# MaaniGhaffari/cvo-rgbd

Measured on AMD Instinct MI355X. Metric: frame-pair registrations/sec, higher is better.
Workload: dtype f32; 1 GPU; BASELINE configs[1] shape: 64 distinct synthetic 10000x10000 RGB-D cloud pairs (xyz + 5-dim colour) per align_many call, cvo align() to convergence, clouds resident in HBM; points_fixed=10000, points_moving=10000, mode=cvo, batch=64

## Files before the change

### cvo-rgbd_amd/csrc/cvo_capi.cpp

```cpp
#include "cvo_internal.h"

using namespace cvo_dev;
using namespace cvo_impl;

namespace cvo_impl {

int fail(cvo_hip_ctx *ctx, int code, const char *msg)
{
    if (ctx) ctx->err = msg;
    return code;
}

static std::atomic<bool> g_engine_debug{false};
bool engine_debug_on() { return g_engine_debug.load(std::memory_order_relaxed); }

namespace {
struct OptDef {
    const char *key;
    const char *env;
    int env_kind;
    double env_value;
};
const OptDef kOptions[] = {
    {"graph_capture", "CVO_HIP_GRAPH", 1, 1.0},           {"no_graph", "CVO_HIP_NO_GRAPH", 1, 1.0},
// ... 822 lines not shown
    else if (is("kept_pack")) *value = !o.no_pack;
    else if (is("matches_combine")) *value = o.matches_combine;
    else if (is("scan_chunk")) *value = o.scan_chunk;
    else if (is("list_margin")) *value = o.list_margin;
    else if (is("record_narrow")) *value = o.record_narrow;
    else if (is("list_stale_max")) *value = o.list_stale_max;
    else if (is("final_mirror")) *value = !o.no_final_mirror;
    else if (is("twist_on_shared_gpu")) *value = o.twist_on_shared_gpu;
    else if (is("comm_debug")) *value = o.comm_debug;
    else if (is("wait_policy")) *value = o.wait_policy;
    else if (is("acvo_runs")) *value = !o.no_acvo_run;
    else if (is("tail_alone")) *value = o.tail_alone;
    else if (is("tail_handovers")) *value = (double)ctx->tail_handovers;
    else if (is("run_restart")) *value = !o.no_restart;
    else if (is("side_builds")) *value = !o.no_side_builds;
    else if (is("run_build_at")) *value = o.run_build_at;
    else if (is("side_builds_launched")) *value = (double)ctx->side_builds_launched;
    else if (is("alone_max")) *value = o.alone_max;
    else if (is("run_timeouts")) *value = (double)ctx->run_timeouts;
    else if (is("list_grows")) *value = (double)ctx->list_grows;
    else if (is("async_builds_named")) *value = (double)ctx->async_stats[0];
    else if (is("async_stalls")) *value = (double)ctx->async_stats[1];
    else if (is("run_aborts")) *value = (double)ctx->run_aborts;
    else if (is("no_run_backoff")) *value = ctx->no_run_backoff;
    else return CVO_HIP_ERR_INVALID;
    return CVO_HIP_OK;
}

long long cvo_hip_get_mirror_retries(void) { return mirror_retries().load(std::memory_order_relaxed); }

int cvo_hip_synchronize(cvo_hip_ctx *ctx)
{
    cvo_lock::Api api_guard;
    if (!ctx) return CVO_HIP_ERR_INVALID;
    HIP_TRY(ctx, hipStreamSynchronize(ctx->stream));
    return CVO_HIP_OK;
}


}
```

### cvo-rgbd_amd/csrc/cvo_device.h

```cpp
#pragma once

#include <hip/hip_runtime.h>
#include <hip/hip_ext.h>
#include <stddef.h>
#include <stdint.h>

#include "cvo_hip.h"
#include "se3_math.hpp"

namespace cvo_dev {

constexpr int FEAT_STRIDE = 8;
constexpr int FEAT_INDEX_SLOT = 5;

constexpr int BLOCK = 256;
constexpr int TILES_PER_WAVE = 4;
constexpr int ROWS_PER_WAVE = 16 * TILES_PER_WAVE;
constexpr int ROWS_PER_TILE = 4 * ROWS_PER_WAVE;
constexpr float PAD_BIG = 1.0e30f;
constexpr int PROC_BLOCKS = 1024;
constexpr int PROC_WAVES = PROC_BLOCKS * 4;

constexpr int NSUB = 256;
constexpr int PROC_PARTS = PROC_BLOCKS / NSUB;
// ... 600 lines not shown
        s->run_hint = (nnz > 0.0f && nnz < 1.0e9f) ? (int32_t)fminf(1.105f * nnz * (q * q) * (w * w), 2.0e9f) : 0;
        s->r_last = r_now;
    }
    if (p.async_self) {
        const float s_xx = reuse_slack(s->t, s->center, s->xmax, s->y0max, 0.0f), s_yy = reuse_slack(s->t, s->center, s->xmax, s->y0max, 1.0f);
        plan_self_async_one<0>(s, p, r_now * 1.0001f + s_xx, p.list_margin, 0.0f, b.sf_fresh[0], b.sf_failed[0], b.sf_inflight[0]);
        plan_self_async_one<1>(s, p, r_now * 1.0001f + s_yy, p.list_margin, s_yy - s_xx, b.sf_fresh[1], b.sf_failed[1], b.sf_inflight[1]);
    }
}

CVO_HD void count_async_plan(DevHead *dst, const DevHead *planned, const DevParams &p)
{
    if (p.async_xy && planned->xy_target >= 0) dst->async_stat[0] += 1;
    if ((p.async_xy || p.async_self) && planned->stall) dst->async_stat[1] += 1;
}

size_t filter_smem_bytes(int jt);
struct PrepareInit {
    int32_t on;
    float R[9], T[3], ell, ell_max;
    int32_t iter, n_fixed, done;
    float center[3], xmax, y0max;
};
struct KeptView {
    const uint2 *kept_ij;
    const float *kept_a;
    const uint32_t *kept_cnt;
    const DevState *st;
    uint32_t kept_wcap;
    int nblk;
    int kept_packed;
    unsigned kept_ebase;
};
#define CVO_GLOBAL __attribute__((address_space(1)))
typedef unsigned u32x2_t __attribute__((ext_vector_type(2)));
typedef float f32x4_t __attribute__((ext_vector_type(4)));
CVO_HD float4 apply_tf(const float *Rt, const float *t, const float4 p)
{
    float4 o;
    o.x = ((Rt[0] * p.x + Rt[1] * p.y) + Rt[2] * p.z) + t[0];
    o.y = ((Rt[3] * p.x + Rt[4] * p.y) + Rt[5] * p.z) + t[1];
    o.z = ((Rt[6] * p.x + Rt[7] * p.y) + Rt[8] * p.z) + t[2];
    o.w = p.w;
    return o;
}

// ... 210 lines not shown
void launch_pose_matches(const MatchArgs &a, bool combine, hipStream_t s);

constexpr int SCAN_TF = 16;
constexpr int SCAN_CHUNK = 4096;
constexpr int SCAN_MAX_POINTS = 65536;
struct ScanArgs {
    const float4 *pos_a;
    const float *feat_a;
    const float4 *seg_a;
    const float4 *pos_b;
    const float *feat_b;
    const float4 *seg_b;
    const float *tf;
    double *partials;
    double *out;
    KernConsts kc;
    int nseg_a, nseg_b;
    int nblk;
    int count;
};
void launch_pose_scan(const ScanArgs &a, int weight, hipStream_t s);

void launch_prepare(DevState *st, const DevParams &prm, hipStream_t s, uint32_t *build_masks = nullptr, const PrepareInit *init = nullptr);
void launch_filter(const FilterArgs &a, dim3 grid, hipStream_t s, hipEvent_t ev_start = nullptr,
                   hipEvent_t ev_stop = nullptr);
void launch_process(int mode, const ProcessArgs &a, hipStream_t s, hipEvent_t ev_start = nullptr,
                    hipEvent_t ev_stop = nullptr);
void launch_post_flow(const PostFlowArgs &a, hipStream_t s);
void launch_post_step(const PostStepArgs &a, hipStream_t s);
void launch_filter_group(const FilterArgs *a, int n, hipStream_t s);
void launch_process_group(int mode, const ProcessArgs *a, int n, hipStream_t s, hipEvent_t ev_start = nullptr,
                          hipEvent_t ev_stop = nullptr);
void launch_post_flow_group(const PostFlowArgs *a, int n, hipStream_t s);
void launch_post_step_group(const PostStepArgs *a, int n, hipStream_t s);
void launch_step_twist_group(const ProcessArgs *a, int n, hipStream_t s, hipEvent_t ev_start = nullptr,
                             hipEvent_t ev_stop = nullptr);
constexpr int STEP_TWIST_ROWS_DIV = 4;

enum TKernel { TK_FILTER = 0, TK_FILTER_GROUP, TK_FLOW, TK_FLOW_MATLAB, TK_STEP, TK_SELF, TK_SELF2, TK_STEP_TWIST,
               TK_FLOW_BUILD, TK_FLOW_BUILD3, TK_FLOW_BUILD6, TK_POST_FLOW, TK_POST_STEP,
               TK_HFLOW_BUILD, TK_HFLOW_BUILD6, TK_HSTEP_TWIST, TK_RUN , TK_RUN_ACVO ,
               TK_SIDE_FILTER, TK_SIDE_RECORD ,
               TK_FLOW_D2  };
constexpr int QP_PARITY = 1 << 8, QP_HEAD = 1 << 9, QP_MASK = 0xff;
struct TLaunch {
    int kernel;
// ... 13 lines not shown
```

### cvo-rgbd_amd/csrc/cvo_engine.cpp

```cpp
#include "cvo_internal.h"

using namespace cvo_dev;
using namespace cvo_impl;

namespace cvo_impl {

bool fusable(const cvo_hip_ctx *c) { return !c->profiling && !multi_rank(c) && !(c->prm.color_scale > 0.0f); }



struct EngineProfile {
    std::mutex mu;
    bool on = false;
    double flow_ms = 0.0, flow_slots = 0.0;
    long long flow_launches = 0;
    std::vector<float> dur_us, period_us;
    std::vector<int> slots;
};
EngineProfile *engine_profile()
{
    static EngineProfile *p = new EngineProfile;
    return p;
}

// ... 10 lines not shown
            (acvo ? !c->allow_async_self : !c->allow_run))
            return false;
        pairs = std::max(pairs, (double)c->fixed.n * (double)c->moving.n);
    }
    const size_t few = acvo ? (pairs <= 1.6e7 ? 12 : (pairs <= 5.0e7 ? 4 : (pairs <= 1.2e8 ? 4 : 0)))
                            : (pairs <= 1.6e7 ? 12 : (pairs <= 5.0e7 ? 8 : (pairs <= 2.0e8 ? 4 : 0)));
    if (const int force = pending.front()->ctx->opt.alone_max) return pending.size() <= (size_t)force;
    return pending.size() <= few;
}

struct Engine {
    int device = 0;
    hipStream_t s = nullptr;
    TableBuf tab;
    PlanCache plans;
    bool in_use = false;

    AlignJob *member[ENGINE_SLOTS] = {};
    std::vector<RecOp> ops[ENGINE_SLOTS];
    Slot slot[ENGINE_SLOTS];
    struct Retire { hipEvent_t ev = nullptr; std::vector<AlignJob *> jobs; };
    std::vector<Retire> retiring;
    hipEvent_t ev[4] = {};
    long long launched = 0, checked = 0;
    int zdim = 0;
    bool crowded = true, use_graph = true, dirty = true, failed = false;
    int batch_len = kEngineBatch;
    bool narrow = false;
    bool narrow_merge = false;
    int narrow_blocks = 0;
    bool wind_down = false;
    std::vector<TLaunch> plan;
    struct FlowEv { hipEvent_t a, b; int live; };
    std::vector<FlowEv> flow_ev;
    long long n_batches[5] = {}, n_replans = 0, n_inserts = 0, n_sends = 0;
    double t_replan = 0, t_insert = 0, t_launch = 0, t_finish = 0, t_wait = 0, t_collect = 0, t_idle_at = 0;
    static double now_ms() { return std::chrono::duration<double, std::milli>(std::chrono::steady_clock::now().time_since_epoch()).count(); }

    int create(int dev)
    {
        device = dev;
        if (hipSetDevice(dev) != hipSuccess) return -1;
        if (hipStreamCreateWithFlags(&s, hipStreamNonBlocking) != hipSuccess) return -1;
        if (tab.init(ENGINE_SLOTS, s) != 0) return -1;
        for (auto &e : ev)
            if (hipEventCreateWithFlags(&e, hipEventDisableTiming) != hipSuccess) return -1;
        return 0;
    }

    int live() const { int n = 0; for (AlignJob *j : member) n += j != nullptr; return n; }
    bool idle() const { return live() == 0 && retiring.empty() && launched == checked; }

    static int nblk_for(int z)
    {
        constexpr int budget = 2048;
        int nblk = 64;
        while (nblk < PROC_BLOCKS && nblk * 2 <= (budget + z / 2) / std::max(1, z)) nblk *= 2;
        return nblk;
// ... 3 lines not shown
    {
        j->rc = rc;
        j->phase = 2;
        j->in_group = false;
        j->ctx->loop_stream = nullptr;
        j->ctx->crowded = false;
        j->ctx->lone = true;
        j->ctx->proc_blocks = j->ctx->proc_blocks_default;
    }

    void fail_all(const char *msg, std::deque<AlignJob *> &pending)
    {
        failed = true;
        (void)hipStreamSynchronize(s);
        for (AlignJob *&j : member)
            if (j) { finish_job(j, fail(j->ctx, CVO_HIP_ERR_HIP, msg)); j = nullptr; }
        for (auto &r : retiring) {
            for (AlignJob *j : r.jobs) finish_job(j, fail(j->ctx, CVO_HIP_ERR_HIP, msg));
            if (r.ev) (void)hipEventDestroy(r.ev);
        }
        retiring.clear();
        for (AlignJob *j : pending) { j->rc = fail(j->ctx, CVO_HIP_ERR_HIP, msg); j->phase = 2; }
        pending.clear();
        for (int z = 0; z < ENGINE_SLOTS; ++z) slot[z].active = 0;
        (void)tab.sync(slot, s, 0);
        (void)hipStreamSynchronize(s);
        launched = checked = 0;
    }

    int insert(AlignJob *j, int z)
    {
        cvo_hip_ctx *c = j->ctx;
        c->loop_stream = s;
        c->crowded = crowded;
        c->lone = false;
        j->in_group = true;
        int rc = CVO_HIP_OK;
        if (j->phase == 3) {
            int32_t zero = 0;
            std::memcpy(&c->st_host[kPollSlots].done, &zero, sizeof(zero));
            if (hipMemcpyAsync(reinterpret_cast<char *>(c->st) + offsetof(DevState, done), &c->st_host[kPollSlots].done,
                               sizeof(zero), hipMemcpyHostToDevice, s) != hipSuccess)
                rc = fail(c, CVO_HIP_ERR_HIP, "resume failed");
            *c->done_mirror = 0;
            launch_prepare(c->st, loop_params(c), s, tab.masks());
            j->phase = 0;
        } else {
            rc = job_begin(*j);
        }
        if (rc) { finish_job(j, rc); return rc; }
        if (j->phase != 0) {
            Retire r;
            if (hipEventCreateWithFlags(&r.ev, hipEventDisableTiming) != hipSuccess || hipEventRecord(r.ev, s) != hipSuccess) {
                finish_job(j, fail(c, CVO_HIP_ERR_HIP, "event failed"));
                return CVO_HIP_ERR_HIP;
            }
            r.jobs.push_back(j);
            retiring.push_back(r);
            return CVO_HIP_OK;
        }
        member[z] = j;
        ops[z].clear();
        dirty = true;
        (void)tab.arm(s);
        return CVO_HIP_OK;
    }

    int replan()
    {
        int n = 0;
        for (int z = 0; z < ENGINE_SLOTS; ++z) n += member[z] != nullptr;
        int zd = 1;
        while (zd < n) zd *= 2;
        if (n > 16 && n <= 24) zd = 24;
        for (int z = ENGINE_SLOTS - 1, hole = 0; z >= zd; --z) {
            if (!member[z]) continue;
            while (member[hole]) ++hole;
            member[hole] = member[z]; member[z] = nullptr;
            ops[hole].swap(ops[z]); ops[z].clear();
        }
        const bool regeom = zd != zdim;
        zdim = zd;
        const int nblk = (narrow && narrow_blocks > 0) ? std::min(narrow_blocks, nblk_for(zdim)) : nblk_for(zdim);
        int merge_max = 2;
        std::vector<const std::vector<RecOp> *> po;
        std::vector<Slot *> ps;
        for (int z = 0; z < ENGINE_SLOTS; ++z)
// ... 9 lines not shown
                c->allow_merge = allow;
                if (rc) return rc;
            }
            std::memset(&slot[z], 0, sizeof(Slot));
            slot[z].active = 1;
            po.push_back(&ops[z]);
            ps.push_back(&slot[z]);
        }
        if (!plan_fused(po, ps, zdim, plan)) return CVO_HIP_ERR_INVALID;
        for (int z = 0; z < ENGINE_SLOTS; ++z)
            if (member[z]) set_build_masks(slot[z], plan, tab.masks(), z);
        const int nq = po.empty() ? 0 : (int)po[0]->size();
        if (tab.sync(slot, s, nq) != 0) return CVO_HIP_ERR_HIP;
        ++n_replans;
        dirty = false;
        return CVO_HIP_OK;
    }

    void collect_stopped()
    {
        Retire r;
        for (int z = 0; z < ENGINE_SLOTS; ++z) {
            AlignJob *j = member[z];
            if (!j || *(volatile int32_t *)j->ctx->done_mirror == RUNNING) continue;
            if (hipMemcpyAsync(&j->ctx->st_host[0], j->ctx->st, sizeof(DevState), hipMemcpyDeviceToHost, s) != hipSuccess) {
                finish_job(j, fail(j->ctx, CVO_HIP_ERR_HIP, "state copy failed"));
            } else {
                r.jobs.push_back(j);
            }
            member[z] = nullptr;
            ops[z].clear();
            dirty = true;
        }
        if (r.jobs.empty()) return;
        if (hipEventCreateWithFlags(&r.ev, hipEventDisableTiming) != hipSuccess || hipEventRecord(r.ev, s) != hipSuccess) {
            for (AlignJob *j : r.jobs) finish_job(j, fail(j->ctx, CVO_HIP_ERR_HIP, "event failed"));
            if (r.ev) (void)hipEventDestroy(r.ev);
            return;
        }
        retiring.push_back(r);
    }

    bool finish_arrived(std::deque<AlignJob *> &pending, bool block)
    {
        bool moved = false;
        while (!retiring.empty()) {
            Retire &r = retiring.front();
            const hipError_t q = block ? hipEventSynchronize(r.ev) : hipEventQuery(r.ev);
            if (q == hipErrorNotReady) break;
            block = false;
// ... 46 lines not shown
                        }
                    }
                    launch_table(tab.dev, l, s);
                }
            return hipGetLastError() == hipSuccess ? CVO_HIP_OK : CVO_HIP_ERR_HIP;
        }
        return run_plan(tab.dev, plans, plan, s, use_graph, batch);
    }

    bool pump(std::deque<AlignJob *> &pending, int want)
    {
        if (failed) return false;
        if (hipSetDevice(device) != hipSuccess) { fail_all("hipSetDevice failed", pending); return true; }
        bool moved = false;
        while (checked < launched) {
            const hipError_t q = hipEventQuery(ev[checked % 4]);
            if (q == hipErrorNotReady) break;
            if (q != hipSuccess) { fail_all("fused poll failed", pending); return true; }
            ++checked;
            { const double t0 = now_ms(); collect_stopped(); t_collect += now_ms() - t0; }
            moved = true;
        }
        { const double t0 = now_ms(); if (finish_arrived(pending, false)) moved = true; t_finish += now_ms() - t0; }
        while (!pending.empty() && live() < std::min(want, (int)ENGINE_SLOTS)) {
            AlignJob *j = pending.front();
            pending.pop_front();
            int z = 0;
            while (member[z]) ++z;
            { const double t0 = now_ms(); insert(j, z); t_insert += now_ms() - t0; }
            moved = true;
        }
        constexpr long long depth = 2;
        while (live() > 0 && launched - checked < depth && !wind_down) {
            if (dirty) {
                const double t0 = now_ms();
                const int rc = replan();
                t_replan += now_ms() - t0;
                if (rc) { fail_all("fused launch recording failed", pending); return true; }
            }
            const double t_l0 = now_ms();
            const int rc_launch = launch_one_batch();
            if (rc_launch != CVO_HIP_OK ||
                hipEventRecord(ev[launched % 4], s) != hipSuccess) {
                fail_all("fused launch failed", pending);
                return true;
            }
            t_launch += now_ms() - t_l0;
            ++launched;
            ++n_batches[zdim >= 16 ? 4 : (zdim >= 8 ? 3 : (zdim >= 4 ? 2 : (zdim >= 2 ? 1 : 0)))];
            moved = true;
        }
        if (live() == 0 && dirty && launched == checked) {
            if (replan() != CVO_HIP_OK) { fail_all("table update failed", pending); return true; }
// ... 58 lines not shown
    if (!e->flow_ev.empty()) {
        EngineProfile *pr = engine_profile();
        std::lock_guard<std::mutex> plock(pr->mu);
        for (size_t q = 0; q < e->flow_ev.size(); ++q) {
            auto &fe = e->flow_ev[q];
            float ms = 0.f, gap = 0.f;
            if (hipEventSynchronize(fe.b) == hipSuccess && hipEventElapsedTime(&ms, fe.a, fe.b) == hipSuccess) {
                pr->flow_ms += ms; pr->flow_launches++; pr->flow_slots += fe.live;
                if (q + 1 < e->flow_ev.size() && hipEventElapsedTime(&gap, fe.a, e->flow_ev[q + 1].a) != hipSuccess) gap = 0.f;
                if (pr->dur_us.size() < (size_t)1 << 20) {
                    pr->dur_us.push_back(ms * 1e3f); pr->period_us.push_back(gap * 1e3f); pr->slots.push_back(fe.live);
                }
            }
        }
        for (auto &fe : e->flow_ev) {
            (void)hipEventDestroy(fe.a);
            (void)hipEventDestroy(fe.b);
        }
        e->flow_ev.clear();
    }
    std::lock_guard<std::mutex> lock(*engine_mutex());
    if (engine_debug_on())
        fprintf(stderr, "[cvo_hip] engine %p: batches at zdim 1/2/4/8/16: %lld %lld %lld %lld %lld, replans %lld, "
                "graph captures %lld hits %lld; host ms: insert %.2f replan %.2f launch %.2f collect %.2f finish %.2f wait %.2f\n",
                (void *)e, e->n_batches[0], e->n_batches[1], e->n_batches[2],
                e->n_batches[3], e->n_batches[4], e->n_replans, e->plans.captures, e->plans.hits,
                e->t_insert, e->t_replan, e->t_launch, e->t_collect, e->t_finish, e->t_wait);
    e->t_insert = e->t_replan = e->t_launch = e->t_collect = e->t_finish = e->t_wait = 0;
    for (long long &v : e->n_batches) v = 0;
    e->n_replans = 0;
    e->launched = e->checked = 0;
    e->in_use = false;
}


}

extern "C" {

int cvo_hip_align_many(cvo_hip_ctx **ctxs, cvo_hip_state **states, int *n_iters, int count)
{
    cvo_lock::Api api_guard;
    if (count < 0 || (count > 0 && (!ctxs || !states))) return CVO_HIP_ERR_INVALID;
    const bool dbg_many = engine_debug_on();
    const double t_many0 = Engine::now_ms();
    struct Tell { double t0; int n; ~Tell() { if (engine_debug_on()) fprintf(stderr, "[cvo_hip] align_many(%d): %.2f ms\n", n, Engine::now_ms() - t0); } } tell{t_many0, count};
    std::vector<AlignJob> jobs((size_t)count);
    for (int i = 0; i < count; ++i) {
        if (!ctxs[i] || !states[i]) return CVO_HIP_ERR_INVALID;
        for (int k = 0; k < i; ++k)
            if (ctxs[k] == ctxs[i]) return CVO_HIP_ERR_INVALID;
        jobs[i].ctx = ctxs[i];
        jobs[i].s = states[i];
// ... 73 lines not shown
                            for (int z = 0; z < ENGINE_SLOTS; ++z) e->ops[z].clear();
                        }
                    if (dbg_many && (left != dbg_left || (int)narrow != dbg_narrow)) { dbg_left = left; dbg_narrow = (int)narrow; fprintf(stderr, "[cvo_hip]   %.2f ms: %d left (narrow %d settled %d)\n", Engine::now_ms() - t_many0, left, (int)narrow, (int)settled); }
                    (void)settled;
                    if (tail_ok && left > 0 && left <= tail_k && narrow) {
                        for (Engine *e : engines) e->wind_down = true;
                        if (dbg_many) {
                            fprintf(stderr, "[cvo_hip]   tail: %d registrations left after %.2f ms, slots done:", left, Engine::now_ms() - t_many0);
                            for (Engine *e : engines)
                                for (AlignJob *j : e->member)
                                    if (j) fprintf(stderr, " %d", *(volatile int32_t *)j->ctx->progress_mirror);
                            fprintf(stderr, "\n");
                        }
                    }
                }
                for (Engine *e : engines) {
                    if (e->wind_down) {
                        const size_t before = leavers.size();
                        e->release_members(leavers);
                        if (leavers.size() != before) {
                            moved = true;
                            if (dbg_many) fprintf(stderr, "[cvo_hip]   tail: %zu registrations leave engine %p after %.2f ms\n", leavers.size() - before, (void *)e, Engine::now_ms() - t_many0);
                        }
                    }
                    if (e->pump(pending, share)) moved = true;
                    if (!e->idle()) any = true;
                    else if (dbg_many && e->t_idle_at == 0) {
                        e->t_idle_at = Engine::now_ms();
                        fprintf(stderr, "[cvo_hip]   engine %p idle after %.2f ms\n", (void *)e, e->t_idle_at - t_many0);
                    }
                }
                if (!any && pending.empty()) break;
                bool alive = false;
                for (Engine *e : engines) alive = alive || !e->failed;
                if (!alive) break;
                if (!moved)
                    for (Engine *e : engines)
                        if (!e->idle() && !e->failed) { e->wait_oldest(pending); break; }
            }
            for (Engine *e : engines) { e->wind_down = false; e->narrow = false; e->batch_len = kEngineBatch; engine_release(e); }
        }
        for (int i = 0; i < count; ++i)
            if (jobs[i].phase == 2 && jobs[i].rc && !first_err) first_err = jobs[i].rc;
    }
    std::vector<char> cont((size_t)count, 0);
    for (AlignJob *j : leavers) {
// ... 92 lines not shown
```

### cvo-rgbd_amd/csrc/cvo_internal.h

```cpp
#pragma once
#include "cvo_hip.h"

#include <hip/hip_runtime.h>

#include <algorithm>
#include <atomic>
#include <chrono>
#include <cmath>
#include <cstddef>
#include <cstdint>
#include <cstdio>
#include <cstdlib>
#include <cstring>
#include <deque>
#include <memory>
#include <mutex>
#include <new>
#include <string>
#include <thread>
#include <vector>

#include "cvo_cloud.h"
#include "cvo_comm.h"
#include "cvo_device.h"
// ... 191 lines not shown
    int tail_alone = 8;
    int alone_max = 0;
    int engines_force = 0;
    int narrow_blocks = 0;
    bool narrow_merge = false;
    int engine_crowd = 2;
    int engine_merge_max = 2;
    double list_init = 0.0;
    float list_margin = -1.0f;
    bool record_narrow = true;
    float list_stale_max = 3.0f;
    int run_cand = 0;
    double mailbox_timeout_s = 5.0;
    double run_timeout_ms = 0.0;
    int run_fault = 0;
    int wait_policy = 0;
};

struct cvo_hip_ctx {
    CtxOptions opt;
    int no_run_backoff = 0;
    long long side_builds_launched = 0;
    long long tail_handovers = 0;
    long long run_aborts = 0;
    int list_stats[3] = {0, 0, 0};
    int async_stats[2] = {0, 0};
    long long list_grows = 0;
    long long run_timeouts = 0;
    int device = 0;
    hipStream_t stream = nullptr;
    bool own_stream = false;
    cvo_hip_params prm{};
    DevParams dprm{};
    Cloud fixed, moving;
    Cloud scratch_a, scratch_b;
    DevState *st = nullptr;
    DevHead *st2 = nullptr;
    bool head_mode = false;
    bool allow_head = true;
    DevState *st_host = nullptr;
    int32_t *done_mirror = nullptr;
    int32_t *progress_mirror = nullptr;
    DevHead *final_mirror = nullptr;
    int32_t *run_mirror = nullptr;
    int32_t *hint_mirror = nullptr;
    int32_t *side_mirror = nullptr;
// ... 146 lines not shown
int enqueue_iterations(cvo_hip_ctx *ctx, int count, int tag0, int trace_cap);
void drop_graphs(cvo_hip_ctx *ctx);
TLaunch mk_launch(int kernel, int q, unsigned gx, unsigned gz, unsigned smem = 0);
bool plan_lone(const std::vector<RecOp> &ops, Slot &slot, std::vector<TLaunch> &plan, const bool allow_head, bool *head_mode,
               std::vector<TLaunch> *pre = nullptr, std::vector<TLaunch> *side = nullptr);
void set_build_masks(Slot &slot, const std::vector<TLaunch> &plan, uint32_t *masks, int z);
bool plan_fused(const std::vector<const std::vector<RecOp> *> &ops, const std::vector<Slot *> &slots, int zdim, std::vector<TLaunch> &plan);
int run_plan(const Slot *tab, PlanCache &cache, const std::vector<TLaunch> &plan, hipStream_t s, bool use_graph, int iterations,
             const std::vector<TLaunch> *pre = nullptr);
int record_iteration(cvo_hip_ctx *ctx, std::vector<RecOp> &ops, int trace_cap);
int prepare_lone_plan(cvo_hip_ctx *ctx, int trace_cap);
int launch_batch(cvo_hip_ctx *ctx, int tag0, int trace_cap, bool with_run = false, int slots = kBatch, bool small_run = false, bool two_runs = false);
constexpr int kNoRunBackoff = 64;
constexpr int kBigRunBackoff = 16;
constexpr int kShortBatch = 2;
constexpr int kRunBatchSlots = 2;
int zero_counters(cvo_hip_ctx *ctx);
int push_state_fields(cvo_hip_ctx *ctx, size_t off, size_t bytes);
int push_pose_fields(cvo_hip_ctx *ctx, const DevHead *img, bool with_consts);
int enqueue_flow_reduce(cvo_hip_ctx *ctx, const CommTable *comm);
int fetch_red(cvo_hip_ctx *ctx, int off, int count, double *out);
void decide_scheme(cvo_hip_ctx *ctx);
std::atomic<long long> &mirror_retries();
int job_begin(AlignJob &j);
int job_finish(AlignJob &j);
int job_continue_alone(AlignJob &j);
int job_pump(AlignJob &j, bool block);

}
```

### cvo-rgbd_amd/csrc/cvo_job.cpp

```cpp
#include "cvo_internal.h"

using namespace cvo_dev;
using namespace cvo_impl;

namespace cvo_impl {

void decide_scheme(cvo_hip_ctx *ctx)
{
    const bool small_pair = (double)ctx->fixed.n * (double)ctx->moving.n <= 2.5e7;
    if (!ctx->proc_blocks_forced)
        ctx->proc_blocks = ctx->proc_blocks_default = small_pair ? PROC_BLOCKS / 2 : PROC_BLOCKS;
    ctx->use_async = ctx->allow_async && !ctx->crowded && !ctx->profiling && !multi_rank(ctx) &&
                     !(ctx->prm.color_scale > 0.0f) &&
                     (double)ctx->fixed.n * (double)ctx->moving.n <= 2.0e8;
    ctx->use_async_self = ctx->use_async && ctx->allow_async_self && ctx->lone &&
                          ctx->prm.mode == CVO_HIP_MODE_ACVO;
    const double npairs = (double)ctx->fixed.n * (double)ctx->moving.n;
    if (ctx->use_async_self && !ctx->proc_blocks_forced)
        ctx->proc_blocks = ctx->proc_blocks_default = npairs <= 6.0e7 ? PROC_BLOCKS / 8 : PROC_BLOCKS / 4;
    if (!ctx->proc_blocks_forced && !ctx->use_async_self && ctx->use_async && ctx->lone && ctx->allow_head &&
        ctx->prm.mode == CVO_HIP_MODE_CVO)
    {
        const bool runs = runs_allowed(ctx) && ctx->fixed.np <= 65536 && ctx->moving.np <= 65536;
        ctx->proc_blocks = ctx->proc_blocks_default =
            npairs <= 2.5e7 ? PROC_BLOCKS / 4 : (npairs <= (runs ? 6.0e7 : 1.5e8) ? PROC_BLOCKS / 2 : PROC_BLOCKS);
    }
}

std::atomic<long long> &mirror_retries()
{
    static std::atomic<long long> n{0};
    return n;
}

int job_begin(AlignJob &j)
{
    cvo_hip_ctx *ctx = j.ctx;
    cvo_hip_state *s = j.s;
    HIP_TRY(ctx, hipSetDevice(ctx->device));
    {
        const int rcm = mailboxes_usable(ctx);
        if (rcm) return rcm;
    }
    const cvo_hip_params &p = ctx->prm;
    if (ctx->no_run_backoff > 0) --ctx->no_run_backoff;
    if (p.mode == CVO_HIP_MODE_ACVO) {
        s->ell = p.ell_init;
        s->ell_max = p.ell_max_init;
    }
    *ctx->done_mirror = 0;
    *ctx->progress_mirror = 0;
    *ctx->run_mirror = 0;
    *ctx->hint_mirror = -1;
    *ctx->side_mirror = 0;
    j.side_seen = 0;
    j.side_launched = 0;
    if (ctx->final_mirror) ctx->final_mirror->done = RUNNING;
    if (!j.trace) j.trace_cap = 0;
// ... 4 lines not shown
        HIP_TRY(ctx, hipMalloc((void **)&ctx->trace_dev, (size_t)j.trace_cap * sizeof(cvo_hip_trace)));
        ctx->trace_dev_cap = j.trace_cap;
    }
    if (j.trace_cap > 0)
        HIP_TRY(ctx, hipMemsetAsync(ctx->trace_dev, 0, (size_t)j.trace_cap * sizeof(cvo_hip_trace),
                                    loop_stream(ctx)));
    PrepareInit in{};
    {
        DevState *h = &ctx->st_host[kPollSlots];
        const int rcg = fill_filter_geometry(ctx, h);
        if (rcg) return rcg;
        in.on = 1;
        std::memcpy(in.R, s->R, sizeof(in.R));
        std::memcpy(in.T, s->T, sizeof(in.T));
        in.ell = s->ell;
        in.ell_max = s->ell_max;
        in.iter = s->iter;
        in.n_fixed = h->n_fixed;
        for (int q = 0; q < 3; ++q) in.center[q] = h->center[q];
        in.xmax = h->xmax; in.y0max = h->y0max;
        in.done = p.max_iter <= 0 ? DONE_MAX_ITER : RUNNING;
    }
    decide_scheme(ctx);
    launch_prepare(ctx->st, loop_params(ctx), loop_stream(ctx), (!j.in_group && ctx->table.raw) ? ctx->table.masks() : nullptr, &in);
    HIP_TRY(ctx, hipGetLastError());
    ctx->have_tf = true;
    const int prc = prepare_buffers(ctx);
    if (prc) return prc;
    ctx->head_mode = false;
    if (!j.in_group && !ctx->profiling && !host_reduce(ctx)) {
        const int rc2 = prepare_lone_plan(ctx, j.trace_cap);
        if (rc2) return rc2;
    }
    j.enq = j.batches = j.checked = 0;
    j.runs_enq = 0;
    j.run_waiting = false;
    j.spec_pending = false;
    j.executed_base = 0;
    const int g_call = std::max(8, std::min(ctx->run_g_max, ctx->run_g_call));
    ctx->run_nnz_max = g_call * RUN_BLOCK * (RUN_R + RUN_L);
    ctx->run_small_max = 3 * RUN_G_SMALL * RUN_BLOCK;
    if (ctx->prm.mode == CVO_HIP_MODE_ACVO) {
        ctx->run_nnz_max = (int)(0.8 * g_call * RUN_BLOCK * RUN_A);
        ctx->run_small_max = (int)(0.8 * 2 * RUN_G_SMALL * RUN_BLOCK);
    }
    if (ctx->big_run_backoff > 0) --ctx->big_run_backoff;
    if (ctx->opt.run_cand > 0) ctx->run_nnz_max = ctx->opt.run_cand;
    j.phase = p.max_iter <= 0 ? 1 : 0;
    if (j.phase == 1) {
        HIP_TRY(ctx, hipMemcpyAsync(&ctx->st_host[0], ctx->st, sizeof(DevState), hipMemcpyDeviceToHost,
                                    loop_stream(ctx)));
        HIP_TRY(ctx, hipEventRecord(ctx->poll_ev[0], loop_stream(ctx)));
    }
    return CVO_HIP_OK;
}

int job_continue_alone(AlignJob &j)
{
    cvo_hip_ctx *ctx = j.ctx;
    HIP_TRY(ctx, hipSetDevice(ctx->device));
    j.in_group = false;
    ctx->loop_stream = nullptr;
    ctx->crowded = false;
    ctx->lone = true;
    ctx->proc_blocks = ctx->proc_blocks_default;
    if (ctx->no_run_backoff > 0) --ctx->no_run_backoff;
    *ctx->done_mirror = 0;
    *ctx->progress_mirror = 0;
    *ctx->run_mirror = 0;
    *ctx->hint_mirror = -1;
    *ctx->side_mirror = 0;
    if (ctx->final_mirror) ctx->final_mirror->done = RUNNING;
    decide_scheme(ctx);
    hipStream_t s = loop_stream(ctx);
    HIP_TRY(ctx, hipMemsetAsync(reinterpret_cast<char *>(ctx->st) + offsetof(DevState, n_slots), 0, sizeof(int32_t), s));
    HIP_TRY(ctx, hipMemsetAsync(reinterpret_cast<char *>(ctx->st) + offsetof(DevState, run_count), 0, 4 * sizeof(int32_t), s));
    HIP_TRY(ctx, hipMemsetAsync(reinterpret_cast<char *>(ctx->st) + offsetof(DevState, run_last_entered), 0, 2 * sizeof(int32_t), s));
    launch_prepare(ctx->st, loop_params(ctx), s, ctx->table.raw ? ctx->table.masks() : nullptr);
    HIP_TRY(ctx, hipGetLastError());
    const int prc = prepare_buffers(ctx);
    if (prc) return prc;
    ctx->head_mode = false;
    const int rc = prepare_lone_plan(ctx, 0);
    if (rc) return rc;
    j.enq = j.batches = j.checked = 0;
    j.runs_enq = 0;
    j.run_waiting = false;
    j.spec_pending = false;
    j.side_seen = 0;
    j.side_launched = 0;
    const int g_call = std::max(8, std::min(ctx->run_g_max, ctx->run_g_call));
    ctx->run_nnz_max = g_call * RUN_BLOCK * (RUN_R + RUN_L);
    ctx->run_small_max = 3 * RUN_G_SMALL * RUN_BLOCK;
    if (ctx->prm.mode == CVO_HIP_MODE_ACVO) {
        ctx->run_nnz_max = (int)(0.8 * g_call * RUN_BLOCK * RUN_A);
        ctx->run_small_max = (int)(0.8 * 2 * RUN_G_SMALL * RUN_BLOCK);
    }
// ... 127 lines not shown
                    continue;
                }
                if (ctx->opt.wait_policy == 0) __builtin_ia32_pause();
                else if (ctx->opt.wait_policy == 1) std::this_thread::yield();
                else std::this_thread::sleep_for(std::chrono::microseconds(50));
                if ((++spins & (ctx->opt.wait_policy == 0 ? 0x3fffu : (ctx->opt.wait_policy == 1 ? 0x3ffu : 0x7u))) == 0u) {
                    const hipError_t q = hipStreamQuery(loop_stream(ctx));
                    if (q != hipSuccess && q != hipErrorNotReady)
                        return finish_with(fail(ctx, CVO_HIP_ERR_HIP, "the stream of the align loop reports an error"));
                    if (q == hipSuccess && *(volatile int32_t *)ctx->done_mirror == RUNNING &&
                        *(volatile int32_t *)ctx->progress_mirror == slots && *(volatile int32_t *)ctx->run_mirror == runs_word) {
                        if (++idle_seen >= 2)
                            return finish_with(fail(ctx, CVO_HIP_ERR_HIP, "the align loop's stream went idle without progress"));
                    } else {
                        idle_seen = 0;
                    }
                }
            }
        }
        {
            const int32_t verdict = *(volatile int32_t *)ctx->done_mirror;
            const bool mirrored = (verdict == DONE_BREAK_A || verdict == DONE_BREAK_B || verdict == DONE_MAX_ITER) && ctx->final_mirror &&
                                  ctx->table.image.size() == 1 && ctx->plan_has_final_mirror;
            if (mirrored) {
                const auto t0 = std::chrono::steady_clock::now();
                for (;;) {
                    std::atomic_thread_fence(std::memory_order_acquire);
                    std::memcpy(&ctx->st_host[0], ctx->final_mirror, sizeof(DevHead));
                    const uint32_t *w = reinterpret_cast<const uint32_t *>(&ctx->st_host[0]);
                    constexpr int pieces = (int)(sizeof(DevHead) / 16);
                    uint32_t sum = 0;
                    for (int q = 0; q < pieces; ++q)
                        sum += head_check_mix(w[4 * q], q == pieces - 1 ? 0u : w[4 * q + 1], w[4 * q + 2], w[4 * q + 3], (unsigned)q);
                    if (ctx->st_host[0].done == verdict && sum == (uint32_t)ctx->st_host[0].head_check_) return finish_with(job_finish(j));
                    mirror_retries().fetch_add(1, std::memory_order_relaxed);
                    if (std::chrono::steady_clock::now() - t0 > std::chrono::microseconds(50)) break;
                    __builtin_ia32_pause();
                }
            }
        }
        if (hipMemcpyAsync(&ctx->st_host[0], ctx->st, sizeof(DevState), hipMemcpyDeviceToHost,
                           ctx->stream) != hipSuccess ||
            hipEventRecord(ctx->poll_ev[0], ctx->stream) != hipSuccess)
            return finish_with(fail(ctx, CVO_HIP_ERR_HIP, "state copy failed"));
        j.phase = 1;
    }
    if (j.phase == 0) {
        bool stop = false;
        while (j.batches - j.checked < 2) {
            int rc = launch_batch(ctx, j.executed_base + j.enq, j.trace_cap);
            if (rc) return finish_with(rc);
            j.enq += kBatch;
            const int slot = j.batches % kPollSlots;
            if (host_reduce(ctx) &&
                hipMemcpyAsync(&ctx->st_host[slot], ctx->st, DEVSTATE_HEAD_BYTES, hipMemcpyDeviceToHost,
                               ctx->stream) != hipSuccess)
                return finish_with(fail(ctx, CVO_HIP_ERR_HIP, "poll copy failed"));
            if (hipEventRecord(ctx->poll_ev[slot], ctx->stream) != hipSuccess)
                return finish_with(fail(ctx, CVO_HIP_ERR_HIP, "poll event failed"));
            ++j.batches;
        }
        const int slot = j.checked % kPollSlots;
// ... 108 lines not shown
```

### cvo-rgbd_amd/csrc/cvo_kernels.hip

```cpp
#include <algorithm>
#include <atomic>
#include <cstdlib>

#include "cvo_device.h"
#include "cvo_pair.h"

namespace cvo_dev {

typedef float f32x4 __attribute__((ext_vector_type(4)));

__device__ __forceinline__ float mv_row(const float *m, float x, float y, float z)
{
    return (m[0] * x + m[1] * y) + m[2] * z;
}

constexpr int FILTER_KMAX = 64;
size_t filter_smem_bytes(int jt)
{
    return (size_t)jt * 16 + ROWS_PER_TILE * 16 + 4 * TILE_STAGE * sizeof(TileEntry) +
           FILTER_KMAX * 4 * 4;
}

__device__ __forceinline__ void flush_tiles(const TileEntry *stage, int n, int lane, unsigned rot, unsigned region,
                                            const FilterArgs &a, int list, TileEntry *tiles, const int par)
// ... 1753 lines not shown
                if (act0) s_st->rec_count[1] = (int32_t)s_cand_total; else s_st->rec_count[0] = (int32_t)s_cand_total;
                if (s_st->stall == 0 && s_st->xy_target < 0 && s_st->xy_fresh < 0) s_st->run_hint = (int32_t)s_cand_total;
            }
            __syncthreads();
        }
        if (publisher) head_prepare_lists<HM>(a, s_st);
    }
    if (publisher) head_publish(a, s_st, out, math);
    return s_st->done == RUNNING && !(async && s_st->stall != 0);
}

__device__ __forceinline__ void post_step_body(const PostStepArgs &a)
{
    __shared__ double sh[4 * NACC_MAX];
    __shared__ __attribute__((aligned(16))) DevHead s_st;
    head_body<HM_CLASSIC>(a, a.st, a.st, &s_st, sh, 0, true);
}

__global__ void __launch_bounds__(BLOCK) k_post_step(const Grp<PostStepArgs> grp)
{
    post_step_body(grp.a[blockIdx.z]);
}

__global__ void k_prepare(DevState *st, const DevParams prm, uint32_t *build_masks, const PrepareInit init)
{
    if (init.on) {
        static_assert(DEVSTATE_INIT_BYTES % 4 == 0, "word stores");
        uint32_t *z = reinterpret_cast<uint32_t *>(st);
        for (int q = threadIdx.x; q < (int)(DEVSTATE_INIT_BYTES / 4); q += BLOCK) z[q] = 0u;
        __syncthreads();
        if (threadIdx.x == 0) {
            for (int q = 0; q < 9; ++q) st->R[q] = init.R[q];
            for (int q = 0; q < 3; ++q) { st->T[q] = init.T[q]; st->center[q] = init.center[q]; }
            st->ell = init.ell; st->ell_max = init.ell_max;
            st->iter = init.iter; st->n_fixed = init.n_fixed; st->done = init.done;
            st->xmax = init.xmax; st->y0max = init.y0max;
        }
        __syncthreads();
    }
    if (build_masks && threadIdx.x < 4) build_masks[threadIdx.x] = 0xffffffffu;
    for (int q = threadIdx.x; q < LIST_N * NSUB; q += BLOCK) (&st->sub[0][0])[q] = 0u;
    if (threadIdx.x < 16) (&st->ovf[0][0])[threadIdx.x] = 0u;
    if (threadIdx.x == 0) {
        for (int l = 0; l < 3; ++l) {
            st->list_ok[l] = 0;
            atomicOr(&st->built[l][(st->k >> 5) & 63], 1u << (st->k & 31));
        }
        for (int l = 0; l < 2; ++l) {
            st->sf_ok[l][0] = st->sf_ok[l][1] = 0;
            st->sf_ck[l][0] = st->sf_ck[l][1] = 0;
            st->sf_active[l] = 0; st->sf_target[l] = -1; st->sf_fresh[l] = -1;
        }
        st->xy_ok[0] = st->xy_ok[1] = 0;
        st->xy_ck[0] = st->xy_ck[1] = 0;
        st->rec_count[0] = st->rec_count[1] = 0;
        st->xy_active = 0;
        st->xy_target = -1;
        st->xy_fresh = -1;
        st->stall = 0;
        st->pending = 0;
        st->mail_snap = st->mail_seq;
        prepare_iteration(st, st, true, prm, plan_builds_none());
        count_async_plan(st, st, prm);
    }
}

void launch_prepare(DevState *st, const DevParams &prm, hipStream_t s, uint32_t *build_masks, const PrepareInit *init)
{
    PrepareInit in{};
    if (init) in = *init;
    hipLaunchKernelGGL(k_prepare, dim3(1), dim3(BLOCK), 0, s, st, prm, build_masks, in);
}

void launch_post_flow_group(const PostFlowArgs *a, int n, hipStream_t s)
{
    Grp<PostFlowArgs> g;
    for (int i = 0; i < n; ++i) g.a[i] = a[i];
    hipLaunchKernelGGL(k_post_flow, dim3(1, 1, (unsigned)n), dim3(BLOCK), 0, s, g);
}

void launch_post_step_group(const PostStepArgs *a, int n, hipStream_t s)
{
    Grp<PostStepArgs> g;
    for (int i = 0; i < n; ++i) g.a[i] = a[i];
    hipLaunchKernelGGL(k_post_step, dim3(1, 1, (unsigned)n), dim3(BLOCK), 0, s, g);
}

typedef const __attribute__((address_space(4))) Slot *CSlot;
#define CVO_SLOT(tab)                          \
    CSlot cs = (CSlot)(tab) + blockIdx.z;      \
    if (cs->active == 0) return
#define CVO_ARG(T, field) (*(const T *)(&cs->field))
#define CVO_FILTER_ROLE(role) (*(const FilterArgs *)(&cs->op[q + (role)].f))

// ... 1519 lines not shown
```

### cvo-rgbd_amd/csrc/cvo_plan.cpp

```cpp
#include "cvo_internal.h"

using namespace cvo_dev;
using namespace cvo_impl;

namespace cvo_impl {

FilterPlan plan_filter(int nrows, int nb)
{
    FilterPlan p{};
    const int tiles = std::max(1, (nrows + ROWS_PER_TILE - 1) / ROWS_PER_TILE);
    const int want_blocks = 4096;
    const int chunks_want = std::max(1, (want_blocks + tiles / 2) / tiles);
    int jt = (nb + chunks_want - 1) / chunks_want;
    jt = std::max(jt, 64);
    jt = std::min(jt, 2048);
    jt = (jt + SEG - 1) & ~(SEG - 1);
    p.jt = jt;
    const int chunks = std::max(1, (nb + jt - 1) / jt);
    p.grid = dim3(chunks, tiles);
    return p;
}

int ensure_buf(cvo_hip_ctx *ctx, DevBuf &b, size_t bytes)
{
// ... 524 lines not shown
            if (fresh) HIP_TRY(ctx, hipMemsetAsync(ctx->run_mail.p, 0, sizeof(RunMail), loop_stream(ctx)));
            pa.run_mail = (RunMail *)ctx->run_mail.p;
            pa.run_mirror = ctx->run_mirror;
            pa.run_iters = 64;
            pa.run_g_max = std::max(8, std::min(ctx->run_g_max, ctx->run_g_call));
            pa.run_timeout_ticks = (long long)(ctx->opt.run_timeout_ms * 1.0e5);
            pa.run_fault = ctx->opt.run_fault;
            if (!ctx->opt.no_side_builds) {
                if (!ctx->side_stream && hipStreamCreateWithFlags(&ctx->side_stream, hipStreamNonBlocking) != hipSuccess) {
                    (void)hipGetLastError();
                    ctx->side_stream = nullptr;
                }
                if (ctx->side_stream) {
                    pa.side_mirror = ctx->side_mirror;
                    pa.run_build_at = ctx->opt.run_build_at;
                }
            }
        } else {
            (void)hipGetLastError();
            ctx->err = "";
        }
    }
    if (ctx->plan_recording && ctx->lone) pa.hint_mirror = ctx->hint_mirror;
    if (ctx->plan_recording && ctx->lone && !multi_rank(ctx) && !ctx->opt.no_final_mirror) pa.final_mirror = ctx->final_mirror;
    if (host_reduce(ctx)) {
        pa.flags = POST_REDUCE;
        emit_post_step(ctx, pa);
        rc = reduce_over_ranks(ctx, RED_STEP, RED_N - RED_STEP);
        if (rc) return rc;
        if (do_math) {
            pa.flags = POST_MATH;
            emit_post_step(ctx, pa);
        }
    } else {
        pa.flags = POST_REDUCE | (do_math ? POST_MATH : 0);
        emit_post_step(ctx, pa);
    }
    HIP_TRY(ctx, hipGetLastError());
    return CVO_HIP_OK;
}

int check_overflow_and_grow(cvo_hip_ctx *ctx, bool *redo)
{
    DevState *h = &ctx->st_host[0];
    HIP_TRY(ctx, hipMemcpyAsync(h->sub, reinterpret_cast<char *>(ctx->st) + offsetof(DevState, sub),
                                sizeof(DevState) - offsetof(DevState, sub), hipMemcpyDeviceToHost,
                                ctx->stream));
// ... 520 lines not shown
```

Baseline: 4332 registrations/s.

## Batch prepare launches in engine and read final state from host mirror

```diff
diff --git a/cvo-rgbd_amd/csrc/cvo_capi.cpp b/cvo-rgbd_amd/csrc/cvo_capi.cpp
--- a/cvo-rgbd_amd/csrc/cvo_capi.cpp
+++ b/cvo-rgbd_amd/csrc/cvo_capi.cpp
@@ -868,6 +868,9 @@
     else if (is("async_builds_named")) *value = (double)ctx->async_stats[0];
     else if (is("async_stalls")) *value = (double)ctx->async_stats[1];
     else if (is("run_aborts")) *value = (double)ctx->run_aborts;
+    else if (is("engine_begins")) *value = (double)ctx->engine_begins;
+    else if (is("engine_final_mirrored")) *value = (double)ctx->engine_final_mirrored;
+    else if (is("engine_final_copied")) *value = (double)ctx->engine_final_copied;
     else if (is("no_run_backoff")) *value = ctx->no_run_backoff;
     else return CVO_HIP_ERR_INVALID;
     return CVO_HIP_OK;
diff --git a/cvo-rgbd_amd/csrc/cvo_device.h b/cvo-rgbd_amd/csrc/cvo_device.h
--- a/cvo-rgbd_amd/csrc/cvo_device.h
+++ b/cvo-rgbd_amd/csrc/cvo_device.h
@@ -646,6 +646,12 @@
     int32_t iter, n_fixed, done;
     float center[3], xmax, y0max;
 };
+struct PrepareEntry {
+    DevState *st;
+    DevParams prm;
+    PrepareInit init;
+};
+static_assert(sizeof(Grp<PrepareEntry>) + 16 <= 4096, "a group of prepare entries and the masks' address must fit the kernel arguments");
 struct KeptView {
     const uint2 *kept_ij;
     const float *kept_a;
@@ -902,6 +908,7 @@
 void launch_pose_scan(const ScanArgs &a, int weight, hipStream_t s);
 
 void launch_prepare(DevState *st, const DevParams &prm, hipStream_t s, uint32_t *build_masks = nullptr, const PrepareInit *init = nullptr);
+void launch_prepare_many(const PrepareEntry *e, int n, hipStream_t s, uint32_t *build_masks);
 void launch_filter(const FilterArgs &a, dim3 grid, hipStream_t s, hipEvent_t ev_start = nullptr,
                    hipEvent_t ev_stop = nullptr);
 void launch_process(int mode, const ProcessArgs &a, hipStream_t s, hipEvent_t ev_start = nullptr,
diff --git a/cvo-rgbd_amd/csrc/cvo_engine.cpp b/cvo-rgbd_amd/csrc/cvo_engine.cpp
--- a/cvo-rgbd_amd/csrc/cvo_engine.cpp
+++ b/cvo-rgbd_amd/csrc/cvo_engine.cpp
@@ -56,6 +56,7 @@
     struct Retire { hipEvent_t ev = nullptr; std::vector<AlignJob *> jobs; };
     std::vector<Retire> retiring;
     hipEvent_t ev[4] = {};
+    std::vector<PrepareEntry> prep;
     long long launched = 0, checked = 0;
     int zdim = 0;
     bool crowded = true, use_graph = true, dirty = true, failed = false;
@@ -67,7 +68,7 @@
     std::vector<TLaunch> plan;
     struct FlowEv { hipEvent_t a, b; int live; };
     std::vector<FlowEv> flow_ev;
-    long long n_batches[5] = {}, n_replans = 0, n_inserts = 0, n_sends = 0;
+    long long n_batches[5] = {}, n_replans = 0, n_inserts = 0, n_sends = 0, n_prepares = 0, n_mirrored = 0, n_copied = 0;
     double t_replan = 0, t_insert = 0, t_launch = 0, t_finish = 0, t_wait = 0, t_collect = 0, t_idle_at = 0;
     static double now_ms() { return std::chrono::duration<double, std::milli>(std::chrono::steady_clock::now().time_since_epoch()).count(); }
 
@@ -117,10 +118,20 @@
         retiring.clear();
         for (AlignJob *j : pending) { j->rc = fail(j->ctx, CVO_HIP_ERR_HIP, msg); j->phase = 2; }
         pending.clear();
+        prep.clear();
         for (int z = 0; z < ENGINE_SLOTS; ++z) slot[z].active = 0;
         (void)tab.sync(slot, s, 0);
         (void)hipStreamSynchronize(s);
         launched = checked = 0;
+    }
+
+    int flush_prepare()
+    {
+        if (prep.empty()) return CVO_HIP_OK;
+        launch_prepare_many(prep.data(), (int)prep.size(), s, tab.masks());
+        n_prepares += ((long long)prep.size() + MAXG - 1) / MAXG;
+        prep.clear();
+        return hipGetLastError() == hipSuccess ? CVO_HIP_OK : CVO_HIP_ERR_HIP;
     }
 
     int insert(AlignJob *j, int z)
@@ -138,15 +149,24 @@
                                sizeof(zero), hipMemcpyHostToDevice, s) != hipSuccess)
                 rc = fail(c, CVO_HIP_ERR_HIP, "resume failed");
             *c->done_mirror = 0;
-            launch_prepare(c->st, loop_params(c), s, tab.masks());
+            PrepareEntry e{};
+            e.st = c->st;
+            e.prm = loop_params(c);
+            if (!rc) prep.push_back(e);
             j->phase = 0;
         } else {
-            rc = job_begin(*j);
+            PrepareEntry e{};
+            rc = job_begin(*j, &e);
+            if (!rc) prep.push_back(e);
         }
         if (rc) { finish_job(j, rc); return rc; }
+        ++c->engine_begins;
         if (j->phase != 0) {
             Retire r;
-            if (hipEventCreateWithFlags(&r.ev, hipEventDisableTiming) != hipSuccess || hipEventRecord(r.ev, s) != hipSuccess) {
+            if (flush_prepare() != CVO_HIP_OK ||
+                hipMemcpyAsync(&c->st_host[0], c->st, sizeof(DevState), hipMemcpyDeviceToHost, s) != hipSuccess ||
+                hipEventCreateWithFlags(&r.ev, hipEventDisableTiming) != hipSuccess || hipEventRecord(r.ev, s) != hipSuccess) {
+                if (r.ev) (void)hipEventDestroy(r.ev);
                 finish_job(j, fail(c, CVO_HIP_ERR_HIP, "event failed"));
                 return CVO_HIP_ERR_HIP;
             }
@@ -157,7 +177,6 @@
         member[z] = j;
         ops[z].clear();
         dirty = true;
-        (void)tab.arm(s);
         return CVO_HIP_OK;
     }
 
@@ -213,10 +232,21 @@
         Retire r;
         for (int z = 0; z < ENGINE_SLOTS; ++z) {
             AlignJob *j = member[z];
-            if (!j || *(volatile int32_t *)j->ctx->done_mirror == RUNNING) continue;
-            if (hipMemcpyAsync(&j->ctx->st_host[0], j->ctx->st, sizeof(DevState), hipMemcpyDeviceToHost, s) != hipSuccess) {
+            if (!j) continue;
+            cvo_hip_ctx *c = j->ctx;
+            const int32_t verdict = *(volatile int32_t *)c->done_mirror;
+            if (verdict == RUNNING) continue;
+            const bool mirrored = (verdict == DONE_BREAK_A || verdict == DONE_BREAK_B || verdict == DONE_MAX_ITER) && c->final_mirror &&
+                                  !c->opt.no_final_mirror && !multi_rank(c);
+            if (mirrored && take_final_mirror(c, verdict)) {
+                ++n_mirrored;
+                ++c->engine_final_mirrored;
+                finish_job(j, job_finish(*j));
+            } else if (hipMemcpyAsync(&j->ctx->st_host[0], j->ctx->st, sizeof(DevState), hipMemcpyDeviceToHost, s) != hipSuccess) {
                 finish_job(j, fail(j->ctx, CVO_HIP_ERR_HIP, "state copy failed"));
             } else {
+                ++n_copied;
+                ++c->engine_final_copied;
                 r.jobs.push_back(j);
             }
             member[z] = nullptr;
@@ -309,13 +339,19 @@
             moved = true;
         }
         { const double t0 = now_ms(); if (finish_arrived(pending, false)) moved = true; t_finish += now_ms() - t0; }
-        while (!pending.empty() && live() < std::min(want, (int)ENGINE_SLOTS)) {
+        while (!wind_down && !pending.empty() && live() < std::min(want, (int)ENGINE_SLOTS)) {
             AlignJob *j = pending.front();
             pending.pop_front();
             int z = 0;
             while (member[z]) ++z;
             { const double t0 = now_ms(); insert(j, z); t_insert += now_ms() - t0; }
             moved = true;
+        }
+        {
+            const double t0 = now_ms();
+            const int rc = flush_prepare();
+            t_insert += now_ms() - t0;
+            if (rc) { fail_all("prepare launch failed", pending); return true; }
         }
         constexpr long long depth = 2;
         while (live() > 0 && launched - checked < depth && !wind_down) {
@@ -420,13 +456,13 @@
     std::lock_guard<std::mutex> lock(*engine_mutex());
     if (engine_debug_on())
         fprintf(stderr, "[cvo_hip] engine %p: batches at zdim 1/2/4/8/16: %lld %lld %lld %lld %lld, replans %lld, "
-                "graph captures %lld hits %lld; host ms: insert %.2f replan %.2f launch %.2f collect %.2f finish %.2f wait %.2f\n",
+                "prepare launches %lld, final states mirrored %lld copied %lld, graph captures %lld hits %lld; host ms: insert %.2f replan %.2f launch %.2f collect %.2f finish %.2f wait %.2f\n",
                 (void *)e, e->n_batches[0], e->n_batches[1], e->n_batches[2],
-                e->n_batches[3], e->n_batches[4], e->n_replans, e->plans.captures, e->plans.hits,
+                e->n_batches[3], e->n_batches[4], e->n_replans, e->n_prepares, e->n_mirrored, e->n_copied, e->plans.captures, e->plans.hits,
                 e->t_insert, e->t_replan, e->t_launch, e->t_collect, e->t_finish, e->t_wait);
     e->t_insert = e->t_replan = e->t_launch = e->t_collect = e->t_finish = e->t_wait = 0;
     for (long long &v : e->n_batches) v = 0;
-    e->n_replans = 0;
+    e->n_replans = e->n_prepares = e->n_mirrored = e->n_copied = 0;
     e->launched = e->checked = 0;
     e->in_use = false;
 }
@@ -546,6 +582,11 @@
                             moved = true;
                             if (dbg_many) fprintf(stderr, "[cvo_hip]   tail: %zu registrations leave engine %p after %.2f ms\n", leavers.size() - before, (void *)e, Engine::now_ms() - t_many0);
                         }
+                        while (!pending.empty()) {
+                            leavers.push_back(pending.front());
+                            pending.pop_front();
+                            moved = true;
+                        }
                     }
                     if (e->pump(pending, share)) moved = true;
                     if (!e->idle()) any = true;
diff --git a/cvo-rgbd_amd/csrc/cvo_internal.h b/cvo-rgbd_amd/csrc/cvo_internal.h
--- a/cvo-rgbd_amd/csrc/cvo_internal.h
+++ b/cvo-rgbd_amd/csrc/cvo_internal.h
@@ -237,6 +237,9 @@
     int no_run_backoff = 0;
     long long side_builds_launched = 0;
     long long tail_handovers = 0;
+    long long engine_begins = 0;
+    long long engine_final_mirrored = 0;
+    long long engine_final_copied = 0;
     long long run_aborts = 0;
     int list_stats[3] = {0, 0, 0};
     int async_stats[2] = {0, 0};
@@ -429,7 +432,8 @@
 int fetch_red(cvo_hip_ctx *ctx, int off, int count, double *out);
 void decide_scheme(cvo_hip_ctx *ctx);
 std::atomic<long long> &mirror_retries();
-int job_begin(AlignJob &j);
+int job_begin(AlignJob &j, PrepareEntry *defer = nullptr);
+bool take_final_mirror(cvo_hip_ctx *ctx, int32_t verdict);
 int job_finish(AlignJob &j);
 int job_continue_alone(AlignJob &j);
 int job_pump(AlignJob &j, bool block);
diff --git a/cvo-rgbd_amd/csrc/cvo_job.cpp b/cvo-rgbd_amd/csrc/cvo_job.cpp
--- a/cvo-rgbd_amd/csrc/cvo_job.cpp
+++ b/cvo-rgbd_amd/csrc/cvo_job.cpp
@@ -33,7 +33,25 @@
     return n;
 }
 
-int job_begin(AlignJob &j)
+bool take_final_mirror(cvo_hip_ctx *ctx, int32_t verdict)
+{
+    const auto t0 = std::chrono::steady_clock::now();
+    for (;;) {
+        std::atomic_thread_fence(std::memory_order_acquire);
+        std::memcpy(&ctx->st_host[0], ctx->final_mirror, sizeof(DevHead));
+        const uint32_t *w = reinterpret_cast<const uint32_t *>(&ctx->st_host[0]);
+        constexpr int pieces = (int)(sizeof(DevHead) / 16);
+        uint32_t sum = 0;
+        for (int q = 0; q < pieces; ++q)
+            sum += head_check_mix(w[4 * q], q == pieces - 1 ? 0u : w[4 * q + 1], w[4 * q + 2], w[4 * q + 3], (unsigned)q);
+        if (ctx->st_host[0].done == verdict && sum == (uint32_t)ctx->st_host[0].head_check_) return true;
+        mirror_retries().fetch_add(1, std::memory_order_relaxed);
+        if (std::chrono::steady_clock::now() - t0 > std::chrono::microseconds(50)) return false;
+        __builtin_ia32_pause();
+    }
+}
+
+int job_begin(AlignJob &j, PrepareEntry *defer)
 {
     cvo_hip_ctx *ctx = j.ctx;
     cvo_hip_state *s = j.s;
@@ -84,8 +102,14 @@
         in.done = p.max_iter <= 0 ? DONE_MAX_ITER : RUNNING;
     }
     decide_scheme(ctx);
-    launch_prepare(ctx->st, loop_params(ctx), loop_stream(ctx), (!j.in_group && ctx->table.raw) ? ctx->table.masks() : nullptr, &in);
-    HIP_TRY(ctx, hipGetLastError());
+    if (defer) {
+        defer->st = ctx->st;
+        defer->prm = loop_params(ctx);
+        defer->init = in;
+    } else {
+        launch_prepare(ctx->st, loop_params(ctx), loop_stream(ctx), (!j.in_group && ctx->table.raw) ? ctx->table.masks() : nullptr, &in);
+        HIP_TRY(ctx, hipGetLastError());
+    }
     ctx->have_tf = true;
     const int prc = prepare_buffers(ctx);
     if (prc) return prc;
@@ -109,7 +133,7 @@
     if (ctx->big_run_backoff > 0) --ctx->big_run_backoff;
     if (ctx->opt.run_cand > 0) ctx->run_nnz_max = ctx->opt.run_cand;
     j.phase = p.max_iter <= 0 ? 1 : 0;
-    if (j.phase == 1) {
+    if (j.phase == 1 && !defer) {
         HIP_TRY(ctx, hipMemcpyAsync(&ctx->st_host[0], ctx->st, sizeof(DevState), hipMemcpyDeviceToHost,
                                     loop_stream(ctx)));
         HIP_TRY(ctx, hipEventRecord(ctx->poll_ev[0], loop_stream(ctx)));
@@ -135,6 +159,12 @@
     if (ctx->final_mirror) ctx->final_mirror->done = RUNNING;
     decide_scheme(ctx);
     hipStream_t s = loop_stream(ctx);
+    if (j.phase == 3) {
+        int32_t zero = 0;
+        std::memcpy(&ctx->st_host[kPollSlots].done, &zero, sizeof(zero));
+        HIP_TRY(ctx, hipMemcpyAsync(reinterpret_cast<char *>(ctx->st) + offsetof(DevState, done), &ctx->st_host[kPollSlots].done, sizeof(zero),
+                                    hipMemcpyHostToDevice, s));
+    }
     HIP_TRY(ctx, hipMemsetAsync(reinterpret_cast<char *>(ctx->st) + offsetof(DevState, n_slots), 0, sizeof(int32_t), s));
     HIP_TRY(ctx, hipMemsetAsync(reinterpret_cast<char *>(ctx->st) + offsetof(DevState, run_count), 0, 4 * sizeof(int32_t), s));
     HIP_TRY(ctx, hipMemsetAsync(reinterpret_cast<char *>(ctx->st) + offsetof(DevState, run_last_entered), 0, 2 * sizeof(int32_t), s));
@@ -308,22 +338,7 @@
             const int32_t verdict = *(volatile int32_t *)ctx->done_mirror;
             const bool mirrored = (verdict == DONE_BREAK_A || verdict == DONE_BREAK_B || verdict == DONE_MAX_ITER) && ctx->final_mirror &&
                                   ctx->table.image.size() == 1 && ctx->plan_has_final_mirror;
-            if (mirrored) {
-                const auto t0 = std::chrono::steady_clock::now();
-                for (;;) {
-                    std::atomic_thread_fence(std::memory_order_acquire);
-                    std::memcpy(&ctx->st_host[0], ctx->final_mirror, sizeof(DevHead));
-                    const uint32_t *w = reinterpret_cast<const uint32_t *>(&ctx->st_host[0]);
-                    constexpr int pieces = (int)(sizeof(DevHead) / 16);
-                    uint32_t sum = 0;
-                    for (int q = 0; q < pieces; ++q)
-                        sum += head_check_mix(w[4 * q], q == pieces - 1 ? 0u : w[4 * q + 1], w[4 * q + 2], w[4 * q + 3], (unsigned)q);
-                    if (ctx->st_host[0].done == verdict && sum == (uint32_t)ctx->st_host[0].head_check_) return finish_with(job_finish(j));
-                    mirror_retries().fetch_add(1, std::memory_order_relaxed);
-                    if (std::chrono::steady_clock::now() - t0 > std::chrono::microseconds(50)) break;
-                    __builtin_ia32_pause();
-                }
-            }
+            if (mirrored && take_final_mirror(ctx, verdict)) return finish_with(job_finish(j));
         }
         if (hipMemcpyAsync(&ctx->st_host[0], ctx->st, sizeof(DevState), hipMemcpyDeviceToHost,
                            ctx->stream) != hipSuccess ||
diff --git a/cvo-rgbd_amd/csrc/cvo_kernels.hip b/cvo-rgbd_amd/csrc/cvo_kernels.hip
--- a/cvo-rgbd_amd/csrc/cvo_kernels.hip
+++ b/cvo-rgbd_amd/csrc/cvo_kernels.hip
@@ -1799,7 +1799,7 @@
     post_step_body(grp.a[blockIdx.z]);
 }
 
-__global__ void k_prepare(DevState *st, const DevParams prm, uint32_t *build_masks, const PrepareInit init)
+__device__ __forceinline__ void prepare_body(DevState *st, const DevParams &prm, uint32_t *build_masks, const PrepareInit &init)
 {
     if (init.on) {
         static_assert(DEVSTATE_INIT_BYTES % 4 == 0, "word stores");
@@ -1842,11 +1842,33 @@
     }
 }
 
+__global__ void k_prepare(DevState *st, const DevParams prm, uint32_t *build_masks, const PrepareInit init)
+{
+    prepare_body(st, prm, build_masks, init);
+}
+
+__global__ void k_prepare_many(const Grp<PrepareEntry> grp, uint32_t *build_masks)
+{
+    const PrepareEntry &e = grp.a[blockIdx.x];
+    prepare_body(e.st, e.prm, blockIdx.x == 0 ? build_masks : nullptr, e.init);
+}
+
 void launch_prepare(DevState *st, const DevParams &prm, hipStream_t s, uint32_t *build_masks, const PrepareInit *init)
 {
     PrepareInit in{};
     if (init) in = *init;
     hipLaunchKernelGGL(k_prepare, dim3(1), dim3(BLOCK), 0, s, st, prm, build_masks, in);
+}
+
+void launch_prepare_many(const PrepareEntry *e, int n, hipStream_t s, uint32_t *build_masks)
+{
+    for (int at = 0; at < n; at += MAXG) {
+        const int m = n - at < MAXG ? n - at : MAXG;
+        Grp<PrepareEntry> g;
+        for (int i = 0; i < m; ++i) g.a[i] = e[at + i];
+        for (int i = m; i < MAXG; ++i) g.a[i] = e[at];
+        hipLaunchKernelGGL(k_prepare_many, dim3((unsigned)m), dim3(BLOCK), 0, s, g, build_masks);
+    }
 }
 
 void launch_post_flow_group(const PostFlowArgs *a, int n, hipStream_t s)
diff --git a/cvo-rgbd_amd/csrc/cvo_plan.cpp b/cvo-rgbd_amd/csrc/cvo_plan.cpp
--- a/cvo-rgbd_amd/csrc/cvo_plan.cpp
+++ b/cvo-rgbd_amd/csrc/cvo_plan.cpp
@@ -570,7 +570,7 @@
         }
     }
     if (ctx->plan_recording && ctx->lone) pa.hint_mirror = ctx->hint_mirror;
-    if (ctx->plan_recording && ctx->lone && !multi_rank(ctx) && !ctx->opt.no_final_mirror) pa.final_mirror = ctx->final_mirror;
+    if (ctx->plan_recording && !multi_rank(ctx) && !ctx->opt.no_final_mirror) pa.final_mirror = ctx->final_mirror;
     if (host_reduce(ctx)) {
         pa.flags = POST_REDUCE;
         emit_post_step(ctx, pa);
```

Result: faster. 4422 registrations/s, median of 6 (+2.1%).
